# sea-with-sakura/ViT-of-Pytorch

Hardware: AMD Instinct MI355X
Metric: images/sec training step, ViT-B/16 224px bf16, 1/2/4/8 MI355X (higher is better)
Workload: dtype bf16; 1 GPU; ViT-B16 @224 train step (fwd+CE+bwd+SGD-momentum/OneCycleLR); model=ViT-B16, image_size=224, per_gpu_batch=256, global_batch=256, seq_len=197, num_classes=1000, parallelism=dp1, step_launch=eager

## Files before the change

### include/vit_hip.h

```cpp
#ifndef VIT_HIP_H_
#define VIT_HIP_H_

#include <stdint.h>

#ifdef __cplusplus
extern "C" {
#endif

typedef void* vit_stream_t;

enum vit_status {
  VIT_OK = 0,
  VIT_ERR_INVALID_ARG = 1,
  VIT_ERR_HIP = 2,
  VIT_ERR_UNSUPPORTED = 3,
};

const char* vit_last_error(void);
int vit_abi_version(void);
const char* vit_build_id(void);

enum vit_layout { VIT_K_CONTIG = 0, VIT_MN_CONTIG = 1 };

typedef struct vit_dropout {
// ... 84 lines not shown
                      const float* mean, const float* rstd, const float* gamma,
                      const float* dres, int64_t lddres, float* dx, int64_t lddx,
                      void* dx_bf16, int64_t lddxb, float* partial, float* dgamma_dbeta,
                      float* dx_colsum, int32_t accumulate_params, int64_t rows, int64_t D,
                      const vit_dropout* dx_dropout, vit_stream_t stream);

int vit_attention_fwd(const void* qkv, void* o, float* lse, int64_t B, int64_t N, int64_t H,
                      int64_t hd, float scale, vit_stream_t stream);
int vit_attention_bwd(const void* qkv, const void* o, const void* dout, const float* lse, void* dqkv,
                      float* bias_partial, int64_t B, int64_t N, int64_t H, int64_t hd, float scale,
                      vit_stream_t stream);
int vit_attention_fwd_rows(const void* qkv, void* o, float* lse, int64_t B, int64_t N, int64_t H, int64_t hd,
                           float scale, int64_t q_rows, vit_stream_t stream);
int vit_attention_bwd_rows(const void* qkv, const void* o, const void* dout, const float* lse, void* dqkv,
                           float* bias_partial, int64_t B, int64_t N, int64_t H, int64_t hd, float scale,
                           int64_t q_rows, vit_stream_t stream);
int64_t vit_attention_bias_rows(int64_t N, int64_t hd, int32_t path);
int64_t vit_attention_workspace_elems(int64_t B, int64_t N, int64_t H, int32_t path);
int vit_attention_fwd_ex(const void* qkv, void* o, float* lse, int64_t B, int64_t N, int64_t H, int64_t hd,
                         float scale, int64_t q_rows, int32_t path, vit_stream_t stream);
int vit_attention_bwd_ex(const void* qkv, const void* o, const void* dout, const float* lse, void* dqkv,
                         float* bias_partial, int64_t B, int64_t N, int64_t H, int64_t hd, float scale,
                         int64_t q_rows, int32_t path, float* workspace, vit_stream_t stream);

int vit_attention_fwd_varlen(const void* q, int64_t ldq, const void* k, int64_t ldk, const void* v, int64_t ldv,
                             void* o, int64_t ldo, const int32_t* cu_q, int64_t B, int64_t max_q, int64_t Nkv,
                             int64_t H, int64_t hd, float scale, vit_stream_t stream);

int vit_im2col(const float* x, void* out, int64_t B, int64_t img, int64_t P, int64_t Kpad,
               vit_stream_t stream);
int vit_im2col_hw(const float* x, void* out, int64_t B, int64_t H, int64_t W, int64_t Ph, int64_t Pw, int64_t Kpad,
                  vit_stream_t stream);

int vit_preprocess_u8(const uint8_t* images, int64_t B, int64_t H, int64_t W, int64_t image_stride,
                      const uint8_t* flips, int64_t out_h, int64_t out_w, const float* mean_std, float* out,
                      vit_stream_t stream);

enum vit_image_layout { VIT_IMAGES_HWC = 0, VIT_IMAGES_CHW = 1 };
int vit_preprocess_u8_gather(const uint8_t* images, int64_t n_images, int32_t layout, int64_t H, int64_t W,
                             int64_t image_stride, const int64_t* index, int64_t B, const uint8_t* flips,
                             int64_t out_h, int64_t out_w, const float* mean_std, float* out,
                             const int64_t* labels_in, int64_t* labels_out, vit_stream_t stream);

int vit_preprocess_u8_ragged(const uint8_t* bytes, int64_t n_bytes, const int64_t* geom, int64_t n_images,
                             const int64_t* index, int64_t B, const uint8_t* flips, int64_t out_h, int64_t out_w,
                             const float* mean_std, float* out, const int64_t* labels_in, int64_t* labels_out,
// ... 132 lines not shown
```

### vit-of-pytorch_amd/vitmi/_lib.py

```python
from __future__ import annotations

import ctypes
import os

_HERE = os.path.dirname(os.path.abspath(__file__))
LIB_PATH = os.environ.get("VITMI_LIB") or os.path.join(_HERE, "libvit_hip.so")

c_i64 = ctypes.c_int64
c_i32 = ctypes.c_int32
c_f32 = ctypes.c_float
c_vp = ctypes.c_void_p

ABI_VERSION = 24

K_CONTIG, MN_CONTIG = 0, 1
(EPI_F32, EPI_BF16, EPI_BIAS_BF16, EPI_BIAS_GELU, EPI_BIAS_RESID_F32, EPI_GELU_BWD, EPI_PATCH, EPI_SPLITK,
 EPI_BIAS_GELU_DGELU, EPI_MUL_BF16) = range(10)


class Dropout(ctypes.Structure):
    _fields_ = [("p", c_f32), ("site", ctypes.c_uint32), ("seed", ctypes.c_uint64), ("offset", ctypes.c_uint64),
                ("row_stride", c_i64)]


# ... 62 lines not shown
    "vit_cls_mse": (c_i32, [c_vp, c_i64, c_vp, c_i64, c_i64, c_i64, c_vp, c_vp, c_vp, c_vp]),
    "vit_cls_mse_bwd": (c_i32, [c_vp, c_i64, c_vp, c_i64, c_i64, c_vp, c_vp]),
    "vit_router_head_fwd": (c_i32, [c_vp, c_vp, c_i32, c_vp, c_i64, c_i64, c_i32, c_i64, c_i32, c_f32, c_vp, c_vp, c_vp,
                                    c_vp, c_vp, c_vp, c_vp]),
    "vit_router_head_bwd": (c_i32, [c_vp, c_vp, c_vp, c_vp, c_vp, c_vp, c_f32, c_i64, c_i64, c_i32, c_i64, c_i32, c_vp,
                                    c_vp]),
    "vit_splitk_reduce": (c_i32, [c_vp, c_i64, c_i64, c_i64, c_i64, c_vp, c_i64, c_i64, c_i32, c_vp]),
    "vit_layernorm_fwd": (c_i32, [c_vp, c_i64, c_vp, c_vp, c_vp, c_i64, c_i32, c_vp, c_vp, c_i64, c_i64, c_f32, c_vp]),
    "vit_layernorm_bwd_partial_rows": (c_i64, [c_i64]),
    "vit_layernorm_bwd_blocks": (c_i64, [c_i64]),
    "vit_layernorm_bwd": (c_i32, [c_vp, c_i64, c_i32, c_vp, c_i64, c_vp, c_vp, c_vp, c_vp, c_i64, c_vp, c_i64,
                                  c_vp, c_i64, c_vp, c_vp, c_vp, c_i32, c_i64, c_i64, ctypes.POINTER(Dropout),
                                  c_vp]),
    "vit_attention_fwd": (c_i32, [c_vp, c_vp, c_vp, c_i64, c_i64, c_i64, c_i64, c_f32, c_vp]),
    "vit_attention_bwd": (c_i32, [c_vp, c_vp, c_vp, c_vp, c_vp, c_vp, c_i64, c_i64, c_i64, c_i64, c_f32, c_vp]),
    "vit_attention_fwd_rows": (c_i32, [c_vp, c_vp, c_vp, c_i64, c_i64, c_i64, c_i64, c_f32, c_i64, c_vp]),
    "vit_attention_bwd_rows": (c_i32, [c_vp, c_vp, c_vp, c_vp, c_vp, c_vp, c_i64, c_i64, c_i64, c_i64, c_f32, c_i64,
                                       c_vp]),
    "vit_attention_bias_rows": (c_i64, [c_i64, c_i64, c_i32]),
    "vit_attention_workspace_elems": (c_i64, [c_i64, c_i64, c_i64, c_i32]),
    "vit_attention_fwd_ex": (c_i32, [c_vp, c_vp, c_vp, c_i64, c_i64, c_i64, c_i64, c_f32, c_i64, c_i32, c_vp]),
    "vit_attention_bwd_ex": (c_i32, [c_vp, c_vp, c_vp, c_vp, c_vp, c_vp, c_i64, c_i64, c_i64, c_i64, c_f32, c_i64,
                                     c_i32, c_vp, c_vp]),
    "vit_im2col": (c_i32, [c_vp, c_vp, c_i64, c_i64, c_i64, c_i64, c_vp]),
    "vit_im2col_hw": (c_i32, [c_vp, c_vp, c_i64, c_i64, c_i64, c_i64, c_i64, c_i64, c_vp]),
    "vit_preprocess_u8": (c_i32, [c_vp, c_i64, c_i64, c_i64, c_i64, c_vp, c_i64, c_i64, c_vp, c_vp, c_vp]),
    "vit_preprocess_u8_gather": (c_i32, [c_vp, c_i64, c_i32, c_i64, c_i64, c_i64, c_vp, c_i64, c_vp, c_i64, c_i64, c_vp,
                                         c_vp, c_vp, c_vp, c_vp]),
    "vit_preprocess_u8_ragged": (c_i32, [c_vp, c_i64, c_vp, c_i64, c_vp, c_i64, c_vp, c_i64, c_i64, c_vp, c_vp, c_vp,
                                         c_vp, c_vp]),
    "vit_preprocess_u8_ragged_crop": (c_i32, [c_vp, c_i64, c_vp, c_i64, c_vp, c_i64, c_vp, c_vp, c_i64, c_i64, c_vp,
                                              c_vp, c_vp, c_vp, c_vp]),
    "vit_mix_batch": (c_i32, [c_vp, c_vp, c_i64, c_i64, c_i64, c_vp, c_vp, c_vp, c_vp]),
    "vit_embed_grad": (c_i32, [c_vp, c_i64, c_i64, c_i64, c_vp, c_vp, c_vp, ctypes.POINTER(Dropout), c_vp]),
    "vit_embed_grad_accum": (c_i32, [c_vp, c_i64, c_i64, c_i64, c_vp, c_vp, c_vp, ctypes.POINTER(Dropout), c_i32,
                                     c_vp]),
    "vit_dropout_mask": (c_i32, [ctypes.POINTER(Dropout), c_i64, c_i64, c_i64, c_vp, c_i64, c_vp]),
    "vit_colsum_partial_rows": (c_i64, [c_i64]),
    "vit_colsum": (c_i32, [c_vp, c_i32, c_i64, c_i64, c_i64, c_vp, c_vp, c_i32, c_vp]),
    "vit_gemm_f32": (c_i32, [c_i64, c_i64, c_i64, c_vp, c_i64, c_i32, c_vp, c_i64, c_i32, c_vp, c_i64, c_vp, c_i32,
                             c_vp]),
    "vit_cross_entropy": (c_i32, [c_vp, c_vp, c_i64, c_i64, c_vp, c_f32, c_vp, c_vp]),
    "vit_cross_entropy_soft": (c_i32, [c_vp, c_vp, c_vp, c_vp, c_f32, c_i64, c_i64, c_vp, c_f32, c_vp, c_vp]),
    "vit_sgd_step": (c_i32, [c_vp, c_vp, c_vp, c_vp, c_i64, c_f32, c_f32, c_f32, c_i32, c_vp]),
    "vit_cast_f32_bf16": (c_i32, [c_vp, c_vp, c_i64, c_vp]),
    "vit_cast_pad_rows": (c_i32, [c_vp, c_i64, c_i64, c_vp, c_i64, c_vp]),
    "vit_axpby": (c_i32, [c_vp, c_vp, c_i64, c_f32, c_f32, c_vp]),
# ... 78 lines not shown
```

### vit-of-pytorch_amd/vitmi/engine.py

```python
from __future__ import annotations

import math
import os
from collections import OrderedDict
from dataclasses import dataclass

import torch

from . import ops, wgrad
from ._lib import (EPI_BF16, EPI_BIAS_BF16, EPI_BIAS_GELU_DGELU, EPI_BIAS_RESID_F32, EPI_MUL_BF16, EPI_PATCH,
                   K_CONTIG, MN_CONTIG)
from .wgrad import Spec

ALIGN = 64


def _rup(x, m):
    return (x + m - 1) // m * m


_NBUF = 2

_WGRAD_TARGET = int(os.environ.get("VIT_WGRAD_TARGET", "256"))

# ... 139 lines not shown
        self.g = [z(Tp, M) for _ in range(L)]
        self.lncls = z(b, D, dt=f)
        self.muf = z(b, dt=f)
        self.rsf = z(b, dt=f)
        self.logits = z(b, cfg.num_classes, dt=f)
        self.dh = z(Tp, D, dt=f)
        self.dhb = [z(Tp, D), z(Tp, D)]
        self.dg = [z(Tp, M), z(Tp, M)]
        self.dyln = z(Tp, D)
        self.dO = z(Tp, D)
        self.dqkv = [z(Tp, 3 * D), z(Tp, 3 * D)]
        self.dlncls = z(b, D, dt=f)
        self.dlogits = z(b, cfg.num_classes, dt=f)
        self.row_stats = z(b, 3, dt=f)
        self.lnparts = [z(ops.layernorm_bwd_blocks(T), 3 * D, dt=f) for _ in range(_NBUF)]
        self.gelu_parts = [z(-(-T // 128), M, dt=f) for _ in range(_NBUF)]
        self.attn_bias_rows = ops.attention_bias_rows(N, D // H)
        self.qkv_bparts = [z(b * self.attn_bias_rows, 3 * D, dt=f) for _ in range(_NBUF)]
        nws = ops.attention_workspace_elems(b, N, H)
        self.attn_ws = z(nws, dt=f) if nws else None
        bp = _rup(b, 64)
        self.bp = bp
        self.c_o, self.c_ln2, self.c_dh, self.c_dh2, self.c_dyln = (z(bp, D) for _ in range(5))
        self.c_g, self.c_gp, self.c_dg = (z(bp, M) for _ in range(3))
        self.c_mu2, self.c_rs2 = z(b, dt=f), z(b, dt=f)
        self._cfg, self._dev = cfg, dev
        self.dhb_l = self.dg_l = self.dqkv_l = None

    def defer_bufs(self):
        if self.dhb_l is None:
            cfg = self._cfg
            D, M, L = cfg.emb_dim, cfg.mlp_dim, cfg.num_layers
            z = lambda *s: torch.zeros(*s, device=self._dev, dtype=torch.bfloat16)
            self.dhb_l = self.dhb + [z(self.Tp, D) for _ in range(2 * L - 1)]
            self.dg_l = self.dg + [z(self.Tp, M) for _ in range(max(L - 2, 0))]
            self.dqkv_l = self.dqkv + [z(self.Tp, 3 * D) for _ in range(max(L - 2, 0))]
        return self.dhb_l, self.dg_l, self.dqkv_l


class _BiasReducer:

    def __init__(self, eng, a, accumulate=False):
        self.eng = eng
        self.a = a
        self.accumulate = accumulate
        self.D = eng.cfg.emb_dim
# ... 101 lines not shown
        D, L = cfg.emb_dim, cfg.num_layers
        M = cfg.mlp_dim
        bf = torch.bfloat16
        self.wqkv = torch.zeros(L, D, 3 * D, device=self.dev, dtype=bf)
        self.bqkv = torch.zeros(L, 3 * D, device=self.dev)
        kp = _rup(cfg.patch_k, 64)
        self.wconv = torch.zeros(D, kp, device=self.dev, dtype=torch.bfloat16) if kp != cfg.patch_k else None
        self._acts = {}
        self._mirror_sig = None
        o = [self.off(self.lname(i, "norm1.weight")) for i in range(L)]
        self.layer_stride = o[0] - o[1] if L > 1 else 0
        assert all(o[i] == o[0] - i * self.layer_stride for i in range(L))
        self._ws = None
        self.step_id = 0
        self.grad_ready_hook = None
        self.grad_ready_finish = None
        self.overlap_wgrad = os.environ.get("VITMI_OVERLAP", "0") == "1"
        self.group_wgrad = os.environ.get("VITMI_GROUP_WGRAD", "1") != "0"
        v = os.environ.get("VITMI_WGRAD_DEFER", "all")
        self.wgrad_defer = L if v == "all" else int(v)
        self._wgrad_tables = {}
        self.prune_last = os.environ.get("VITMI_PRUNE_LAST", "1") != "0"
        self._pruned = False
        self._side = None
        self._ev_pool, self._ev_next = [], 0
        self.probe = None
        self.probe_wgrad = None
        self.drop_seed = (torch.initial_seed() * 0x9E3779B97F4A7C15 + 0x632BE59BD9B4E019) & (2**64 - 1)
        self._drop_offset = 0
        self._drop = None

    def _event(self):
        if self._ev_next == len(self._ev_pool):
            self._ev_pool.append(torch.cuda.Event())
        ev = self._ev_pool[self._ev_next]
        self._ev_next += 1
        return ev

    def pv(self, name, buf=None):
        return self.layout.view(self.flat if buf is None else buf, name)

    def off(self, name):
        return self.layout.offsets[name]

    def lname(self, i, s):
        return f"transformer.encoder_layers.{i}.{s}"
# ... 55 lines not shown
        b = x.shape[0]
        a = self.acts(b)
        D, M, H, N, L = cfg.emb_dim, cfg.mlp_dim, cfg.num_heads, cfg.tokens, cfg.num_layers
        hd = D // H
        T = a.T
        mv = self.mirror
        f = self.flat
        if dropout_p and dropout_p > 0.0:
            if not dropout_p < 1.0:
                raise ValueError(f"dropout probability has to be in [0, 1), got {dropout_p}")
            self._drop_offset += 1
            self._drop = (float(dropout_p), self.drop_seed, self._drop_offset)
        else:
            self._drop = None
        dd = self._dd
        ops.im2col_hw(x, a.patches, b, *cfg.image_hw, *cfg.patch_hw, a.kpad)
        wconv = self.wconv if self.wconv is not None else mv[self.off("embedding.weight"):]
        ops.gemm(a.patches, wconv, a.h[0], T, D, a.kpad, a_layout=K_CONTIG, b_layout=K_CONTIG, lda=a.kpad,
                 ldb=a.kpad, ldc=D, epilogue=EPI_PATCH, bias=f[self.off("embedding.bias"):],
                 aux=f[self.off("transformer.pos_embedding.pos_embedding"):], ldaux=D,
                 aux2=f[self.off("cls_token"):], tokens=N, dropout=dd(0))
        scale = 1.0 / math.sqrt(hd)
        self._pruned = self.prune_last and self._drop is None
        for i in range(L):
            ln = lambda s: self.off(self.lname(i, s))
            ops.layernorm_fwd(a.h[i], D, f[ln("norm1.weight"):], f[ln("norm1.bias"):], a.ln1[i], D, a.mu1[i],
                              a.rs1[i], T, D)
            ops.gemm(a.ln1[i], self.wqkv[i], a.qkv[i], T, 3 * D, D, a_layout=K_CONTIG, b_layout=MN_CONTIG, lda=D,
                     ldb=3 * D, ldc=3 * D, epilogue=EPI_BIAS_BF16, bias=self.bqkv[i])
            last = self._pruned and i == L - 1
            ops.attention_fwd(a.qkv[i], a.o[i], a.lse[i], b, N, H, hd, scale, q_rows=1 if last else None,
                              path=self.attn_fwd_path)
            if last:
                self._forward_last_cls(a, i, b)
                break
            ops.gemm(a.o[i], mv[ln("attn.out.weight"):], a.hm[i], T, D, D, a_layout=K_CONTIG, b_layout=MN_CONTIG,
                     lda=D, ldb=D, ldc=D, epilogue=EPI_BIAS_RESID_F32, bias=f[ln("attn.out.bias"):], aux=a.h[i],
                     ldaux=D, dropout=dd(1 + 3 * i))
            ops.layernorm_fwd(a.hm[i], D, f[ln("norm2.weight"):], f[ln("norm2.bias"):], a.ln2[i], D, a.mu2[i],
                              a.rs2[i], T, D)
            wgrad.timed(self.probe, (), ops.gemm, a.ln2[i], mv[ln("mlp.fc1.weight"):], a.gp[i], T, M, D,
                        a_layout=K_CONTIG, b_layout=K_CONTIG, lda=D, ldb=D, ldc=M, epilogue=EPI_BIAS_GELU_DGELU,
                        bias=f[ln("mlp.fc1.bias"):], C2=a.g[i], ldc2=M, dropout=dd(2 + 3 * i))
            ops.gemm(a.g[i], mv[ln("mlp.fc2.weight"):], a.h[i + 1], T, D, M, a_layout=K_CONTIG, b_layout=K_CONTIG,
                     lda=M, ldb=M, ldc=D, epilogue=EPI_BIAS_RESID_F32, bias=f[ln("mlp.fc2.bias"):], aux=a.hm[i],
                     ldaux=D, dropout=dd(3 + 3 * i))
        ops.layernorm_fwd(a.h[L], N * D, f[self.off("transformer.norm.weight"):], f[self.off("transformer.norm.bias"):],
                          a.lncls, D, a.muf, a.rsf, b, D)
        C = cfg.num_classes
        ops.gemm_f32(b, C, D, a.lncls, D, False, f[self.off("classifier.weight"):], D, True, a.logits, C,
                     bias=f[self.off("classifier.bias"):])
        self.step_id += 1
        self._last_b = b
        return a.logits

# ... 14 lines not shown
                 lda=M, ldb=M, ldc=S, epilogue=EPI_BIAS_RESID_F32, bias=f[ln("mlp.fc2.bias"):], aux=a.hm[i], ldaux=S)

    def _backward_last_cls(self, a, i, b, g, wq, bias):
        cfg = self.cfg
        D, M, N = cfg.emb_dim, cfg.mlp_dim, cfg.tokens
        S = N * D
        f, mv = self.flat, self.mirror
        gv = lambda name: g[self.off(self.lname(i, name)):]
        bp = a.bp
        wq.single(Spec(a.c_dh, D, a.c_g, M, D, M, gv("mlp.fc2.weight"), M), K=bp)
        gpart = bias.buf("gelu", a.gelu_parts)
        w2 = mv[self.off(self.lname(i, "mlp.fc2.weight")):]
        kw = dict(a_layout=K_CONTIG, b_layout=MN_CONTIG, lda=D, ldb=M, ldc=M, epilogue=EPI_MUL_BF16, aux=a.c_gp,
                  ldaux=M, col_partial=gpart)
        ops.gemm(a.c_dh, w2, a.c_dg, b, M, D, **kw)
        tiles_m = ops.gemm_partial_rows(a.c_dh, w2, a.c_dg, b, M, D, **kw)
        bias.reduce(gpart, tiles_m, M, M, (gv("mlp.fc1.bias"),))
        wq.single(Spec(a.c_dg, M, a.c_ln2, D, M, D, gv("mlp.fc1.weight"), D), K=bp)
        ops.gemm(a.c_dg, mv[self.off(self.lname(i, "mlp.fc1.weight")):], a.c_dyln, b, D, M, a_layout=K_CONTIG,
                 b_layout=MN_CONTIG, lda=M, ldb=D, ldc=D, epilogue=EPI_BF16)
        bias.ln_bwd(a.c_dyln, D, a.hm[i], S, a.c_mu2, a.c_rs2, f[self.off(self.lname(i, "norm2.weight")):], a.dh, S, b,
                    gv("norm2.weight"), gv("attn.out.bias"), dres=a.dh, lddres=S, dx_bf16=a.c_dh2, lddxb=D)
        wq.single(Spec(a.c_o, D, a.c_dh2, D, D, D, gv("attn.out.weight"), D), K=bp)
        ops.zero_(a.dO)
        ops.gemm(a.c_dh2, mv[self.off(self.lname(i, "attn.out.weight")):], a.dO, b, D, D, a_layout=K_CONTIG,
                 b_layout=K_CONTIG, lda=D, ldb=D, ldc=S, epilogue=EPI_BF16)

    def forward_exact(self, x: torch.Tensor):
        cfg = self.cfg
        if x.dim() != 4 or x.shape[1] != 3 or tuple(x.shape[2:]) != cfg.image_hw:
            raise ValueError(f"expected input [b, 3, {cfg.image_hw[0]}, {cfg.image_hw[1]}], got {tuple(x.shape)}")
        x = x.to(self.dev, torch.float32).contiguous()
        b = x.shape[0]
        D, M, H, N, L, C = cfg.emb_dim, cfg.mlp_dim, cfg.num_heads, cfg.tokens, cfg.num_layers, cfg.num_classes
        hd = D // H
        T, kp = b * N, cfg.patch_k
        f = self.flat
        e = lambda *shape: torch.empty(*shape, device=self.dev)
        fv = lambda name: f[self.off(name):]
        patches = e(T, kp)
        ops.im2col_hw_f32(x, patches, b, *cfg.image_hw, *cfg.patch_hw, kp)
        h = e(T, D)
        ops.gemm_f32(T, D, kp, patches, kp, False, fv("embedding.weight"), kp, True, h, D, bias=fv("embedding.bias"))
        ops.embed_fwd_f32(h, b, N, D, fv("transformer.pos_embedding.pos_embedding"), fv("cls_token"))
        y, qkv, o, u = e(T, D), e(T, 3 * D), e(T, D), e(T, M)
        mu, rs = e(T), e(T)
        for i in range(L):
# ... 120 lines not shown
                w2 = mv[ln("mlp.fc2.weight"):]
                kw = dict(a_layout=K_CONTIG, b_layout=MN_CONTIG, lda=D, ldb=M, ldc=M, epilogue=EPI_MUL_BF16, aux=a.gp[i],
                          ldaux=M, col_partial=gpart)
                ops.gemm(dhb, w2, dg, T, M, D, **kw)
                tiles_m = ops.gemm_partial_rows(dhb, w2, dg, T, M, D, **kw)
                bias.reduce(gpart, tiles_m, M, M, (gv(self.lname(i, "mlp.fc1.bias")),))
                wq.push(Spec(dg, M, a.ln2[i], D, M, D, gv(self.lname(i, "mlp.fc1.weight")), D),
                        done=lambda k=li: release("dg", k))
                ops.gemm(dg, mv[ln("mlp.fc1.weight"):], a.dyln, T, D, M, a_layout=K_CONTIG, b_layout=MN_CONTIG, lda=M,
                         ldb=D, ldc=D, epilogue=EPI_BF16)
                wb = (wb + 1) % nd
                acquire("dhb", wb)
                dhb = dhbs[wb]
                bias.ln_bwd(a.dyln, D, a.hm[i], D, a.mu2[i], a.rs2[i], f[ln("norm2.weight"):], a.dh, D, T,
                            gv(self.lname(i, "norm2.weight")), gv(self.lname(i, "attn.out.bias")),
                            dres=a.dh, lddres=D, dx_bf16=dhb, lddxb=D, dx_dropout=dd(1 + 3 * i))
                wq.push(Spec(a.o[i], D, dhb, D, D, D, gv(self.lname(i, "attn.out.weight")), D),
                        done=lambda k=wb: release("dhb", k), hold=True)
                ops.gemm(dhb, mv[ln("attn.out.weight"):], a.dO, T, D, D, a_layout=K_CONTIG, b_layout=K_CONTIG, lda=D,
                         ldb=D, ldc=D, epilogue=EPI_BF16)
            dqkv = dqkvs[li]
            acquire("dqkv", li)
            qpart = bias.buf("qkv", a.qkv_bparts)
            ops.attention_bwd(a.qkv[i], a.o[i], a.dO, a.lse[i], dqkv, b, N, H, hd, scale, bias_partial=qpart,
                              q_rows=1 if pruned and i == L - 1 else None, workspace=a.attn_ws)
            qo = ln("attn.query.weight")
            zs = ln("attn.key.weight") - qo
            qb = ln("attn.query.bias")
            bias.reduce(qpart, b * a.attn_bias_rows, 3 * D, 3 * D, (g[qb:], g[qb + zs:], g[qb + 2 * zs:]), seg=D)
            wq.push(Spec(a.ln1[i], D, dqkv, 3 * D, D, D, g[qo:], D, batch=3, b_bs=D, out_bs=zs),
                    done=lambda k=li: release("dqkv", k))
            wq.end_layer(i)
            ops.gemm(dqkv, self.wqkv[i], a.dyln, T, D, 3 * D, a_layout=K_CONTIG, b_layout=K_CONTIG, lda=3 * D,
                     ldb=3 * D, ldc=D, epilogue=EPI_BF16)
            wb = (wb + 1) % nd
            acquire("dhb", wb)
            bias.ln_bwd(a.dyln, D, a.h[i], D, a.mu1[i], a.rs1[i], f[ln("norm1.weight"):], a.dh, D, T,
                        gv(self.lname(i, "norm1.weight")), gv(self.lname(i - 1, "mlp.fc2.bias")) if i > 0 else None,
                        dres=a.dh, lddres=D, dx_bf16=dhbs[wb], lddxb=D,
                        dx_dropout=dd(3 + 3 * (i - 1)) if i > 0 else dd(0))
            fire(self.layout.buckets[L - i])
        wq.push(Spec(dhbs[wb], D, a.patches, a.kpad, D, cfg.patch_k, gv("embedding.weight"), cfg.patch_k))
        wq.finish()
        ops.embed_grad(a.dh, b, N, D, gv("transformer.pos_embedding.pos_embedding"), gv("cls_token"),
                       gv("embedding.bias"), dropout=dd(0), accumulate=accumulate)
        fire(self.layout.buckets[-1])
        bias.flush()
        if overlap:
            main.wait_stream(side)
        return g
```

### vit-of-pytorch_amd/vitmi/ops.py

```python
from __future__ import annotations

import ctypes

import torch

from . import _lib
from ._lib import COLSUM_BATCH_MAX, Dropout, GemmArgs, check

BF16 = torch.bfloat16
F32 = torch.float32


def lib():
    return _lib.load()


def _stream():
    return ctypes.c_void_p(torch.cuda.current_stream().cuda_stream)


def _p(t):
    return ctypes.c_void_p(0 if t is None else t.data_ptr())


# ... 124 lines not shown
def attention_workspace_elems(B, N, H, path=ATTN_AUTO):
    return int(lib().vit_attention_workspace_elems(B, N, H, path))


def attention_fwd(qkv, o, lse, B, N, H, hd, scale, q_rows=None, path=ATTN_AUTO):
    _chk(qkv, BF16, "qkv")
    _chk(o, BF16, "o")
    _chk(lse, F32, "lse")
    check(lib().vit_attention_fwd_ex(_p(qkv), _p(o), _p(lse), B, N, H, hd, scale, N if q_rows is None else q_rows,
                                     path, _stream()), "vit_attention_fwd")


def attention_bwd(qkv, o, dout, lse, dqkv, B, N, H, hd, scale, bias_partial=None, q_rows=None, path=ATTN_AUTO,
                  workspace=None):
    _chk(workspace, F32, "workspace")
    need = attention_workspace_elems(B, N, H, path)
    if need and (workspace is None or workspace.numel() < need):
        if workspace is not None:
            raise ValueError(f"attention workspace has {workspace.numel()} floats, needs {need}")
        workspace = torch.empty(need, device=qkv.device, dtype=F32)
    check(lib().vit_attention_bwd_ex(_p(qkv), _p(o), _p(dout), _p(lse), _p(dqkv), _p(bias_partial), B, N, H, hd,
                                     scale, N if q_rows is None else q_rows, path, _p(workspace if need else None),
                                     _stream()), "vit_attention_bwd")


def im2col(x, out, B, img, P, Kpad):
    _chk(x, F32, "x")
    _chk(out, BF16, "out")
    check(lib().vit_im2col(_p(x), _p(out), B, img, P, Kpad, _stream()), "vit_im2col")


def im2col_hw(x, out, B, H, W, Ph, Pw, Kpad):
    _chk(x, F32, "x")
    _chk(out, BF16, "out")
    check(lib().vit_im2col_hw(_p(x), _p(out), B, H, W, Ph, Pw, Kpad, _stream()), "vit_im2col_hw")


def preprocess_u8(images, out, flips=None, mean=(0.5, 0.5, 0.5), std=(0.5, 0.5, 0.5)):
    _chk(images, torch.uint8, "images")
    _chk(out, F32, "out")
    _chk(flips, torch.uint8, "flips")
    if images.dim() != 4 or images.shape[3] != 3 or out.dim() != 4 or out.shape[1] != 3:
        raise ValueError(f"preprocess_u8: images [B,H,W,3] -> out [B,3,h,w], got {tuple(images.shape)} -> "
                         f"{tuple(out.shape)}")
    B, H, W, _ = images.shape
    if out.shape[0] != B or (flips is not None and flips.numel() != B):
# ... 399 lines not shown

def adamw_ema_update(p, g, m, v, p_bf16, ema, chunks, table, lr, beta1, beta2, eps, wd, ema_decay, write_grad):
    for t, name in ((p, "p"), (g, "g"), (m, "m"), (v, "v"), (ema, "ema"), (table, "table")):
        _chk(t, F32, name)
    _chk(p_bf16, BF16, "p_bf16")
    if chunks.is_cuda or chunks.dtype != torch.int64 or not chunks.is_contiguous() or not chunks.is_pinned():
        raise ValueError("adamw_ema_update: chunks must be a contiguous int64 tensor in pinned host memory")
    check(lib().vit_adamw_ema_update(_p(p), _p(g), _p(m), _p(v), _p(p_bf16), _p(ema), _p(chunks), chunks.numel() // 3,
                                     _p(table), 1.0 - lr * wd, beta1, beta2, 1.0 - beta1, 1.0 - beta2, eps,
                                     0.0 if ema is None else 1.0 - ema_decay, int(write_grad), _stream()),
          "vit_adamw_ema_update")


def scale_by_coef(g, n, coef):
    check(lib().vit_scale_by_coef(_p(g), n, _p(coef), _stream()), "vit_scale_by_coef")


def zero_(t):
    if not t.is_contiguous():
        raise ValueError("zero_: contiguous tensor expected")
    check(lib().vit_zero(_p(t), t.numel() * t.element_size(), _stream()), "vit_zero")


def _splitk_model(tiles, slots, tile, K, slab_elems):
    smax = max(1, min((K // 64) // 8, 32))
    t_tile = 2.0 * tile * tile * K / 4.0e12
    slab = 2.0 * slab_elems * 4 / 5.0e12
    best, best_t = 1, None
    for s in range(1, smax + 1):
        t = -(-tiles * s // slots) * t_tile / s + s * slab
        if best_t is None or t < best_t * (1 - 1e-9):
            best, best_t = s, t
    return best


def splitk_factor_group(shapes, K, cus=256):
    tiles = sum(-(-M // 256) * -(-N // 256) * b for M, N, b in shapes)
    return _splitk_model(tiles, cus, 256, K, sum(M * N * b for M, N, b in shapes))


def gemm_splitk_group(members):
    if not 1 <= len(members) <= 4:
        raise ValueError("gemm_splitk_group: 1 to 4 members")
    arr = (GemmArgs * len(members))()
    for i, (A, B, C, M, N, K, kw) in enumerate(members):
        _chk(A, BF16, "A")
        _chk(B, BF16, "B")
        arr[i] = _gemm_args(A, B, C, M, N, K, **kw)
    check(lib().vit_gemm_splitk_group(arr, len(members), _stream()), "vit_gemm_splitk_group")


GEMM_TABLE_MAX = 128


class GemmGroupTable:

    def __init__(self, members):
        n = len(members)
        if not 1 <= n <= GEMM_TABLE_MAX:
            raise ValueError(f"GemmGroupTable: 1 to {GEMM_TABLE_MAX} members")
        arr = (GemmArgs * n)()
# ... 48 lines not shown
```

### vit-of-pytorch_amd/vitmi/wgrad.py

```python
from __future__ import annotations

from typing import NamedTuple

import torch

from . import ops
from ._lib import EPI_SPLITK, MN_CONTIG


class Spec(NamedTuple):
    A: torch.Tensor
    lda: int
    B: torch.Tensor
    ldb: int
    M: int
    N: int
    out: object
    ldo: int
    batch: int = 1
    a_bs: int = 0
    b_bs: int = 0
    out_bs: int = 0
    accumulate: object = False

# ... 58 lines not shown
        jobs += _reduce_jobs(sp, s, w)
    return views, members, jobs


def single(sp, K, alloc=None, target=256, probe=None):
    s = ops.splitk_factor(sp.M, sp.N, K, sp.batch, target)
    ws = _alloc(alloc, sp, _slabs([sp], [s]))
    timed(probe, _tail(probe, [sp], K, False), ops.gemm, sp.A, sp.B, ws, sp.M, sp.N, K, **_gemm_kw(sp, s, sp.N))
    for job in _reduce_jobs(sp, s, ws):
        ops.splitk_reduce(*job)


def group(specs, K, common, alloc=None, target=256, probe=None):
    if common:
        splits = [ops.splitk_factor_group([(sp.M, sp.N, sp.batch) for sp in specs], K, target)] * len(specs)
    else:
        splits = [ops.splitk_factor(sp.M, sp.N, K, sp.batch, target) for sp in specs]
    _, members, jobs = plan(specs, K, splits, _alloc(alloc, specs[0], _slabs(specs, splits)))
    timed(probe, _tail(probe, specs, K, True), ops.gemm_splitk_group, members)
    ops.splitk_reduce_group(jobs)


def table(specs, K, tables, slot, alloc=None, target=256, probe=None):
    s = ops.splitk_factor_group([(sp.M, sp.N, sp.batch) for sp in specs], K, target)
    ws = _alloc(alloc, specs[0], _slabs(specs, [s] * len(specs))) if s > 1 else None
    jobs, o = [], 0
    for c0 in range(0, len(specs), ops.GEMM_TABLE_MAX):
        part = specs[c0:c0 + ops.GEMM_TABLE_MAX]
        key = (s, K, o, ws.data_ptr() if s > 1 else 0) + tuple(
            (sp.A.data_ptr(), sp.lda, sp.B.data_ptr(), sp.ldb, sp.M, sp.N, sp.out.data_ptr(), sp.ldo, sp.batch, sp.a_bs,
             sp.b_bs, sp.out_bs, bool(sp.accumulate)) for sp in part)
        ent = tables.get((slot, c0))
        if ent is None or ent[0] != key:
            _, members, red = plan(part, K, [s] * len(part), ws[o:] if s > 1 else None, table=True)
            ent = tables[(slot, c0)] = (key, ops.GemmGroupTable(members), red)
        timed(probe, _tail(probe, part, K, True), ent[1].launch)
        jobs += ent[2]
        o += _slabs(part, [s] * len(part)) if s > 1 else 0
    if jobs:
        ops.splitk_reduce_group(jobs)
```

Baseline: 7761 images/sec.

## Prune last-layer Q projection to CLS rows with dedicated CLS attention kernels

In the last transformer layer, only the CLS token's output is needed, so the QKV projection now computes K and V for all tokens but Q only for the CLS row. New single-query attention forward and backward kernels handle that layer. The backward pass likewise restricts the Q weight-gradient and the dX GEMM to the CLS rows, and drops the dO zeroing. Separately, the split-K cost model for table wgrad no longer charges a reduction slab when split is 1. The cost is new kernels and copy2d staging, plus dependence on the layout of the existing buffers.

```diff
diff --git a/include/vit_hip.h b/include/vit_hip.h
--- a/include/vit_hip.h
+++ b/include/vit_hip.h
@@ -130,6 +130,13 @@
 int vit_attention_bwd_ex(const void* qkv, const void* o, const void* dout, const float* lse, void* dqkv,
                          float* bias_partial, int64_t B, int64_t N, int64_t H, int64_t hd, float scale,
                          int64_t q_rows, int32_t path, float* workspace, vit_stream_t stream);
+
+int vit_attention_cls_supported(int64_t N, int64_t hd);
+int vit_attention_cls_fwd(const void* qkv, void* o, float* lse, int64_t B, int64_t N, int64_t H, int64_t hd,
+                          float scale, vit_stream_t stream);
+int vit_attention_cls_bwd(const void* qkv, const void* dout, const float* lse, void* dqkv, float* bias_partial,
+                          int64_t bias_rows, int64_t B, int64_t N, int64_t H, int64_t hd, float scale,
+                          vit_stream_t stream);
 
 int vit_attention_fwd_varlen(const void* q, int64_t ldq, const void* k, int64_t ldk, const void* v, int64_t ldv,
                              void* o, int64_t ldo, const int32_t* cu_q, int64_t B, int64_t max_q, int64_t Nkv,
diff --git a/vit-of-pytorch_amd/csrc/attention_cls.hip b/vit-of-pytorch_amd/csrc/attention_cls.hip
--- /dev/null
+++ b/vit-of-pytorch_amd/csrc/attention_cls.hip
@@ -0,0 +1,317 @@
+#include "common.h"
+
+namespace {
+
+constexpr int TPB = 256;
+constexpr int QPAD = 96;
+constexpr int64_t MAX_N = 1024;
+
+__device__ __forceinline__ void unpack8(const uint4& w, float* f) {
+  f[0] = __uint_as_float(w.x << 16); f[1] = __uint_as_float(w.x & 0xffff0000u);
+  f[2] = __uint_as_float(w.y << 16); f[3] = __uint_as_float(w.y & 0xffff0000u);
+  f[4] = __uint_as_float(w.z << 16); f[5] = __uint_as_float(w.z & 0xffff0000u);
+  f[6] = __uint_as_float(w.w << 16); f[7] = __uint_as_float(w.w & 0xffff0000u);
+}
+__device__ __forceinline__ float dot8(const uint4& w, const float* x) {
+  float f[8];
+  unpack8(w, f);
+  float s = f[0] * x[0];
+#pragma unroll
+  for (int e = 1; e < 8; ++e) s = fmaf(f[e], x[e], s);
+  return s;
+}
+__device__ __forceinline__ float round_bf(float x) { return bf2f(f2bf(x)); }
+
+__device__ __forceinline__ float block_sum(float v, float* red) {
+  v = wave_sum(v);
+  if ((threadIdx.x & 63) == 0) red[threadIdx.x >> 6] = v;
+  __syncthreads();
+  const float r = (red[0] + red[1]) + (red[2] + red[3]);
+  __syncthreads();
+  return r;
+}
+__device__ __forceinline__ float block_max(float v, float* red) {
+  v = wave_max(v);
+  if ((threadIdx.x & 63) == 0) red[threadIdx.x >> 6] = v;
+  __syncthreads();
+  const float r = fmaxf(fmaxf(red[0], red[1]), fmaxf(red[2], red[3]));
+  __syncthreads();
+  return r;
+}
+
+template <int HD>
+struct Geo {
+  static constexpr int CPK = HD / 8;
+  static constexpr int G = TPB / CPK;
+};
+template <int HD>
+size_t part_floats(int N) {
+  const size_t a = (size_t)N * Geo<HD>::CPK, b = (size_t)Geo<HD>::G * HD;
+  return a > b ? a : b;
+}
+inline int pad4(int n) { return (n + 3) & ~3; }
+
+template <int HD>
+__global__ __launch_bounds__(TPB) void attn_cls_fwd_kernel(const bf16_t* __restrict__ qkv, bf16_t* __restrict__ o,
+                                                           float* __restrict__ lse, int N, int npad, int H,
+                                                           float scale) {
+  constexpr int CPK = Geo<HD>::CPK, G = Geo<HD>::G;
+  extern __shared__ __attribute__((aligned(16))) float smem[];
+  float* qs = smem;
+  float* red = qs + QPAD;
+  float* sc = red + 8;
+  float* part = sc + npad;
+  const int tid = threadIdx.x, b = blockIdx.x / H, h = blockIdx.x % H;
+  const int D = H * HD;
+  const size_t ld = 3 * (size_t)D;
+  const bf16_t* base = qkv + (size_t)b * N * ld + (size_t)h * HD;
+  if (tid < HD) qs[tid] = bf2f(base[tid]);
+  __syncthreads();
+  const int g = tid / CPK, c = tid % CPK;
+  const bool active = g < G;
+  float qr[8];
+#pragma unroll
+  for (int e = 0; e < 8; ++e) qr[e] = qs[c * 8 + e];
+  if (active) {
+    const bf16_t* kp = base + D + c * 8;
+#pragma unroll 4
+    for (int j = g; j < N; j += G) {
+      const uint4 w = *reinterpret_cast<const uint4*>(kp + (size_t)j * ld);
+      part[j * CPK + c] = dot8(w, qr);
+    }
+  }
+  __syncthreads();
+  float m = -INFINITY;
+  for (int j = tid; j < N; j += TPB) {
+    float s = part[j * CPK];
+#pragma unroll
+    for (int k = 1; k < CPK; ++k) s += part[j * CPK + k];
+    s *= scale;
+    sc[j] = s;
+    m = fmaxf(m, s);
+  }
+  m = block_max(m, red);
+  float l = 0.0f;
+  for (int j = tid; j < N; j += TPB) {
+    const float p = expf(sc[j] - m);
+    l += p;
+    sc[j] = round_bf(p);
+  }
+  l = block_sum(l, red);
+  float acc[8] = {0.0f, 0.0f, 0.0f, 0.0f, 0.0f, 0.0f, 0.0f, 0.0f};
+  if (active) {
+    const bf16_t* vp = base + 2 * D + c * 8;
+#pragma unroll 4
+    for (int j = g; j < N; j += G) {
+      const uint4 w = *reinterpret_cast<const uint4*>(vp + (size_t)j * ld);
+      float v[8];
+      unpack8(w, v);
+      const float p = sc[j];
+#pragma unroll
+      for (int e = 0; e < 8; ++e) acc[e] = fmaf(p, v[e], acc[e]);
+    }
+#pragma unroll
+    for (int e = 0; e < 8; ++e) part[g * HD + c * 8 + e] = acc[e];
+  }
+  __syncthreads();
+  if (tid < HD) {
+    float s = part[tid];
+    for (int k = 1; k < G; ++k) s += part[k * HD + tid];
+    o[(size_t)b * N * D + (size_t)h * HD + tid] = f2bf(s / l);
+  }
+  if (tid == 0) lse[((size_t)b * H + h) * N] = m + logf(l);
+}
+
+template <int HD>
+__global__ __launch_bounds__(TPB) void attn_cls_bwd_kernel(const bf16_t* __restrict__ qkv,
+                                                           const bf16_t* __restrict__ dout,
+                                                           const float* __restrict__ lse, bf16_t* __restrict__ dqkv,
+                                                           float* __restrict__ bias_partial, int bias_rows, int N,
+                                                           int npad, int H, float scale) {
+  constexpr int CPK = Geo<HD>::CPK, G = Geo<HD>::G;
+  extern __shared__ __attribute__((aligned(16))) float smem[];
+  float* qs = smem;
+  float* dos = qs + QPAD;
+  float* red = dos + QPAD;
+  float* sp = red + 8;
+  float* sd = sp + npad;
+  float* partp = sd + npad;
+  float* parts = partp + (size_t)N * CPK;
+  const int tid = threadIdx.x, b = blockIdx.x / H, h = blockIdx.x % H;
+  const int D = H * HD;
+  const size_t ld = 3 * (size_t)D;
+  const size_t row0 = (size_t)b * N * ld + (size_t)h * HD;
+  const bf16_t* base = qkv + row0;
+  if (tid < HD) {
+    qs[tid] = bf2f(base[tid]);
+    dos[tid] = bf2f(dout[(size_t)b * N * D + (size_t)h * HD + tid]);
+  }
+  const float L = lse[((size_t)b * H + h) * N];
+  __syncthreads();
+  const int g = tid / CPK, c = tid % CPK;
+  const bool active = g < G;
+  float qr[8], dr[8];
+#pragma unroll
+  for (int e = 0; e < 8; ++e) {
+    qr[e] = qs[c * 8 + e];
+    dr[e] = dos[c * 8 + e];
+  }
+  const bf16_t* kp = base + D + c * 8;
+  if (active) {
+#pragma unroll 4
+    for (int j = g; j < N; j += G) {
+      const uint4 kw = *reinterpret_cast<const uint4*>(kp + (size_t)j * ld);
+      const uint4 vw = *reinterpret_cast<const uint4*>(kp + D + (size_t)j * ld);
+      parts[j * CPK + c] = dot8(kw, qr);
+      partp[j * CPK + c] = dot8(vw, dr);
+    }
+  }
+  __syncthreads();
+  float dl = 0.0f;
+  for (int j = tid; j < N; j += TPB) {
+    float s = parts[j * CPK], dp = partp[j * CPK];
+#pragma unroll
+    for (int k = 1; k < CPK; ++k) {
+      s += parts[j * CPK + k];
+      dp += partp[j * CPK + k];
+    }
+    const float p = expf(s * scale - L);
+    sp[j] = p;
+    sd[j] = dp;
+    dl = fmaf(p, dp, dl);
+  }
+  const float delta = block_sum(dl, red);
+  float sum_p = 0.0f, sum_ds = 0.0f;
+  for (int j = tid; j < N; j += TPB) {
+    const float p = sp[j];
+    const float pb = round_bf(p), dsb = round_bf(p * (sd[j] - delta));
+    sp[j] = pb;
+    sd[j] = dsb;
+    sum_p += pb;
+    sum_ds += dsb;
+  }
+  sum_p = block_sum(sum_p, red);
+  sum_ds = block_sum(sum_ds, red);
+  float acc[8] = {0.0f, 0.0f, 0.0f, 0.0f, 0.0f, 0.0f, 0.0f, 0.0f};
+  if (active) {
+    bf16_t* dkp = dqkv + row0 + D + c * 8;
+#pragma unroll 2
+    for (int j = g; j < N; j += G) {
+      const uint4 kw = *reinterpret_cast<const uint4*>(kp + (size_t)j * ld);
+      float k[8];
+      unpack8(kw, k);
+      const float pb = sp[j], dsb = sd[j];
+      uint4 dk, dv;
+      dk.x = pack2bf(scale * (dsb * qr[0]), scale * (dsb * qr[1]));
+      dk.y = pack2bf(scale * (dsb * qr[2]), scale * (dsb * qr[3]));
+      dk.z = pack2bf(scale * (dsb * qr[4]), scale * (dsb * qr[5]));
+      dk.w = pack2bf(scale * (dsb * qr[6]), scale * (dsb * qr[7]));
+      dv.x = pack2bf(pb * dr[0], pb * dr[1]);
+      dv.y = pack2bf(pb * dr[2], pb * dr[3]);
+      dv.z = pack2bf(pb * dr[4], pb * dr[5]);
+      dv.w = pack2bf(pb * dr[6], pb * dr[7]);
+      *reinterpret_cast<uint4*>(dkp + (size_t)j * ld) = dk;
+      *reinterpret_cast<uint4*>(dkp + D + (size_t)j * ld) = dv;
+#pragma unroll
+      for (int e = 0; e < 8; ++e) acc[e] = fmaf(dsb, k[e], acc[e]);
+    }
+#pragma unroll
+    for (int e = 0; e < 8; ++e) parts[g * HD + c * 8 + e] = acc[e];
+  }
+  __syncthreads();
+  if (tid < HD) {
+    float s = parts[tid];
+    for (int k = 1; k < G; ++k) s += parts[k * HD + tid];
+    const float dq = scale * s;
+    dqkv[row0 + tid] = f2bf(dq);
+    if (bias_partial) {
+      float* bp = bias_partial + (size_t)b * bias_rows * ld + (size_t)h * HD + tid;
+      bp[0] = dq;
+      bp[D] = scale * (sum_ds * qs[tid]);
+      bp[2 * D] = sum_p * dos[tid];
+      for (int r = 1; r < bias_rows; ++r) {
+        bp[r * ld] = 0.0f;
+        bp[r * ld + D] = 0.0f;
+        bp[r * ld + 2 * D] = 0.0f;
+      }
+    }
+  }
+}
+
+template <int HD>
+hipError_t launch_fwd(const void* qkv, void* o, float* lse, int B, int N, int H, float scale, hipStream_t s) {
+  const int npad = pad4(N);
+  const size_t lds = (QPAD + 8 + npad + part_floats<HD>(N)) * sizeof(float);
+  auto kern = attn_cls_fwd_kernel<HD>;
+  if (lds > 64 * 1024) (void)hipFuncSetAttribute((const void*)kern, hipFuncAttributeMaxDynamicSharedMemorySize, (int)lds);
+  hipLaunchKernelGGL(kern, dim3(B * H), dim3(TPB), lds, s, (const bf16_t*)qkv, (bf16_t*)o, lse, N, npad, H, scale);
+  return hipGetLastError();
+}
+
+template <int HD>
+hipError_t launch_bwd(const void* qkv, const void* dout, const float* lse, void* dqkv, float* bias_partial,
+                      int bias_rows, int B, int N, int H, float scale, hipStream_t s) {
+  const int npad = pad4(N);
+  const size_t lds = (2 * QPAD + 8 + 2 * npad + (size_t)N * Geo<HD>::CPK + part_floats<HD>(N)) * sizeof(float);
+  auto kern = attn_cls_bwd_kernel<HD>;
+  if (lds > 64 * 1024) (void)hipFuncSetAttribute((const void*)kern, hipFuncAttributeMaxDynamicSharedMemorySize, (int)lds);
+  hipLaunchKernelGGL(kern, dim3(B * H), dim3(TPB), lds, s, (const bf16_t*)qkv, (const bf16_t*)dout, lse, (bf16_t*)dqkv,
+                     bias_partial, bias_rows, N, npad, H, scale);
+  return hipGetLastError();
+}
+
+bool supported(int64_t N, int64_t hd) { return (hd == 32 || hd == 64 || hd == 80) && N >= 1 && N <= MAX_N; }
+bool aligned16(const void* p) { return ((uintptr_t)p & 15) == 0; }
+
+int check(const char* what, int64_t B, int64_t N, int64_t H, int64_t hd) {
+  VIT_CHECK_ARG(B >= 1 && H >= 1 && N >= 1 && hd >= 1, "%s: bad sizes B=%lld N=%lld H=%lld hd=%lld", what, (long long)B,
+                (long long)N, (long long)H, (long long)hd);
+  VIT_CHECK_ARG(B * H <= 0x7fffffff && H * hd <= (1 << 20), "%s: B=%lld H=%lld hd=%lld too large", what, (long long)B,
+                (long long)H, (long long)hd);
+  if (!supported(N, hd)) {
+    vit::set_error("%s: N=%lld hd=%lld unsupported (hd 32, 64 or 80, N <= %lld)", what, (long long)N, (long long)hd,
+                   (long long)MAX_N);
+    return VIT_ERR_UNSUPPORTED;
+  }
+  return VIT_OK;
+}
+
+}
+
+extern "C" int vit_attention_cls_supported(int64_t N, int64_t hd) { return supported(N, hd) ? 1 : 0; }
+
+extern "C" int vit_attention_cls_fwd(const void* qkv, void* o, float* lse, int64_t B, int64_t N, int64_t H, int64_t hd,
+                                     float scale, vit_stream_t stream) {
+  const int st = check("vit_attention_cls_fwd", B, N, H, hd);
+  if (st) return st;
+  VIT_CHECK_ARG(qkv && o && lse, "vit_attention_cls_fwd: null pointer");
+  VIT_CHECK_ARG(aligned16(qkv), "vit_attention_cls_fwd: qkv must be 16-byte aligned");
+  hipStream_t s = (hipStream_t)stream;
+  hipError_t e;
+  switch (hd) {
+    case 32: e = launch_fwd<32>(qkv, o, lse, (int)B, (int)N, (int)H, scale, s); break;
+    case 64: e = launch_fwd<64>(qkv, o, lse, (int)B, (int)N, (int)H, scale, s); break;
+    default: e = launch_fwd<80>(qkv, o, lse, (int)B, (int)N, (int)H, scale, s); break;
+  }
+  return vit::check_hip(e, "vit_attention_cls_fwd launch");
+}
+
+extern "C" int vit_attention_cls_bwd(const void* qkv, const void* dout, const float* lse, void* dqkv,
+                                     float* bias_partial, int64_t bias_rows, int64_t B, int64_t N, int64_t H,
+                                     int64_t hd, float scale, vit_stream_t stream) {
+  const int st = check("vit_attention_cls_bwd", B, N, H, hd);
+  if (st) return st;
+  VIT_CHECK_ARG(qkv && dout && lse && dqkv, "vit_attention_cls_bwd: null pointer");
+  VIT_CHECK_ARG(aligned16(qkv) && aligned16(dqkv), "vit_attention_cls_bwd: qkv / dqkv must be 16-byte aligned");
+  VIT_CHECK_ARG(!bias_partial || (bias_rows >= 1 && bias_rows <= 1024), "vit_attention_cls_bwd: bias_rows=%lld",
+                (long long)bias_rows);
+  hipStream_t s = (hipStream_t)stream;
+  const int br = (int)bias_rows;
+  hipError_t e;
+  switch (hd) {
+    case 32: e = launch_bwd<32>(qkv, dout, lse, dqkv, bias_partial, br, (int)B, (int)N, (int)H, scale, s); break;
+    case 64: e = launch_bwd<64>(qkv, dout, lse, dqkv, bias_partial, br, (int)B, (int)N, (int)H, scale, s); break;
+    default: e = launch_bwd<80>(qkv, dout, lse, dqkv, bias_partial, br, (int)B, (int)N, (int)H, scale, s); break;
+  }
+  return vit::check_hip(e, "vit_attention_cls_bwd launch");
+}
diff --git a/vit-of-pytorch_amd/vitmi/_lib.py b/vit-of-pytorch_amd/vitmi/_lib.py
--- a/vit-of-pytorch_amd/vitmi/_lib.py
+++ b/vit-of-pytorch_amd/vitmi/_lib.py
@@ -108,7 +108,10 @@
     "vit_attention_fwd_ex": (c_i32, [c_vp, c_vp, c_vp, c_i64, c_i64, c_i64, c_i64, c_f32, c_i64, c_i32, c_vp]),
     "vit_attention_bwd_ex": (c_i32, [c_vp, c_vp, c_vp, c_vp, c_vp, c_vp, c_i64, c_i64, c_i64, c_i64, c_f32, c_i64,
                                      c_i32, c_vp, c_vp]),
-    "vit_im2col": (c_i32, [c_vp, c_vp, c_i64, c_i64, c_i64, c_i64, c_vp]),
+    "vit_attention_cls_supported": (c_i32, [c_i64, c_i64]),
+    "vit_attention_cls_fwd": (c_i32, [c_vp, c_vp, c_vp, c_i64, c_i64, c_i64, c_i64, c_f32, c_vp]),
+    "vit_attention_cls_bwd": (c_i32, [c_vp, c_vp, c_vp, c_vp, c_vp, c_i64, c_i64, c_i64, c_i64, c_i64, c_f32, c_vp]),
+    "vit_im2col":(c_i32, [c_vp, c_vp, c_i64, c_i64, c_i64, c_i64, c_vp]),
     "vit_im2col_hw": (c_i32, [c_vp, c_vp, c_i64, c_i64, c_i64, c_i64, c_i64, c_i64, c_vp]),
     "vit_preprocess_u8": (c_i32, [c_vp, c_i64, c_i64, c_i64, c_i64, c_vp, c_i64, c_i64, c_vp, c_vp, c_vp]),
     "vit_preprocess_u8_gather": (c_i32, [c_vp, c_i64, c_i32, c_i64, c_i64, c_i64, c_vp, c_i64, c_vp, c_i64, c_i64, c_vp,
diff --git a/vit-of-pytorch_amd/vitmi/engine.py b/vit-of-pytorch_amd/vitmi/engine.py
--- a/vit-of-pytorch_amd/vitmi/engine.py
+++ b/vit-of-pytorch_amd/vitmi/engine.py
@@ -185,6 +185,7 @@
         bp = _rup(b, 64)
         self.bp = bp
         self.c_o, self.c_ln2, self.c_dh, self.c_dh2, self.c_dyln = (z(bp, D) for _ in range(5))
+        self.c_ln1, self.c_dq = z(bp, D), z(bp, D)
         self.c_g, self.c_gp, self.c_dg = (z(bp, M) for _ in range(3))
         self.c_mu2, self.c_rs2 = z(b, dt=f), z(b, dt=f)
         self._cfg, self._dev = cfg, dev
@@ -332,6 +333,8 @@
         self._wgrad_tables = {}
         self.prune_last = os.environ.get("VITMI_PRUNE_LAST", "1") != "0"
         self._pruned = False
+        self.prune_q = os.environ.get("VITMI_PRUNE_Q", "1") != "0"
+        self._prune_q = False
         self._side = None
         self._ev_pool, self._ev_next = [], 0
         self.probe = None
@@ -433,15 +436,23 @@
                  aux2=f[self.off("cls_token"):], tokens=N, dropout=dd(0))
         scale = 1.0 / math.sqrt(hd)
         self._pruned = self.prune_last and self._drop is None
+        self._prune_q = self._pruned and self.prune_q and ops.attention_cls_supported(N, hd)
         for i in range(L):
             ln = lambda s: self.off(self.lname(i, s))
             ops.layernorm_fwd(a.h[i], D, f[ln("norm1.weight"):], f[ln("norm1.bias"):], a.ln1[i], D, a.mu1[i],
                               a.rs1[i], T, D)
-            ops.gemm(a.ln1[i], self.wqkv[i], a.qkv[i], T, 3 * D, D, a_layout=K_CONTIG, b_layout=MN_CONTIG, lda=D,
-                     ldb=3 * D, ldc=3 * D, epilogue=EPI_BIAS_BF16, bias=self.bqkv[i])
             last = self._pruned and i == L - 1
-            ops.attention_fwd(a.qkv[i], a.o[i], a.lse[i], b, N, H, hd, scale, q_rows=1 if last else None,
-                              path=self.attn_fwd_path)
+            if last and self._prune_q:
+                kw = dict(a_layout=K_CONTIG, b_layout=MN_CONTIG, ldb=3 * D, epilogue=EPI_BIAS_BF16)
+                ops.gemm(a.ln1[i], self.wqkv[i].view(-1)[D:], a.qkv[i].view(-1)[D:], T, 2 * D, D, lda=D, ldc=3 * D,
+                         bias=self.bqkv[i][D:], **kw)
+                ops.gemm(a.ln1[i], self.wqkv[i], a.qkv[i], b, D, D, lda=N * D, ldc=3 * N * D, bias=self.bqkv[i], **kw)
+                ops.attention_cls_fwd(a.qkv[i], a.o[i], a.lse[i], b, N, H, hd, scale)
+            else:
+                ops.gemm(a.ln1[i], self.wqkv[i], a.qkv[i], T, 3 * D, D, a_layout=K_CONTIG, b_layout=MN_CONTIG, lda=D,
+                         ldb=3 * D, ldc=3 * D, epilogue=EPI_BIAS_BF16, bias=self.bqkv[i])
+                ops.attention_fwd(a.qkv[i], a.o[i], a.lse[i], b, N, H, hd, scale, q_rows=1 if last else None,
+                                  path=self.attn_fwd_path)
             if last:
                 self._forward_last_cls(a, i, b)
                 break
@@ -502,7 +513,8 @@
         bias.ln_bwd(a.c_dyln, D, a.hm[i], S, a.c_mu2, a.c_rs2, f[self.off(self.lname(i, "norm2.weight")):], a.dh, S, b,
                     gv("norm2.weight"), gv("attn.out.bias"), dres=a.dh, lddres=S, dx_bf16=a.c_dh2, lddxb=D)
         wq.single(Spec(a.c_o, D, a.c_dh2, D, D, D, gv("attn.out.weight"), D), K=bp)
-        ops.zero_(a.dO)
+        if not self._prune_q:
+            ops.zero_(a.dO)
         ops.gemm(a.c_dh2, mv[self.off(self.lname(i, "attn.out.weight")):], a.dO, b, D, D, a_layout=K_CONTIG,
                  b_layout=K_CONTIG, lda=D, ldb=D, ldc=S, epilogue=EPI_BF16)
 
@@ -669,17 +681,33 @@
             dqkv = dqkvs[li]
             acquire("dqkv", li)
             qpart = bias.buf("qkv", a.qkv_bparts)
-            ops.attention_bwd(a.qkv[i], a.o[i], a.dO, a.lse[i], dqkv, b, N, H, hd, scale, bias_partial=qpart,
-                              q_rows=1 if pruned and i == L - 1 else None, workspace=a.attn_ws)
+            pq = self._prune_q and i == L - 1
+            if pq:
+                ops.attention_cls_bwd(a.qkv[i], a.dO, a.lse[i], dqkv, b, N, H, hd, scale, bias_partial=qpart,
+                                      bias_rows=a.attn_bias_rows)
+            else:
+                ops.attention_bwd(a.qkv[i], a.o[i], a.dO, a.lse[i], dqkv, b, N, H, hd, scale, bias_partial=qpart,
+                                  q_rows=1 if pruned and i == L - 1 else None, workspace=a.attn_ws)
             qo = ln("attn.query.weight")
             zs = ln("attn.key.weight") - qo
             qb = ln("attn.query.bias")
             bias.reduce(qpart, b * a.attn_bias_rows, 3 * D, 3 * D, (g[qb:], g[qb + zs:], g[qb + 2 * zs:]), seg=D)
-            wq.push(Spec(a.ln1[i], D, dqkv, 3 * D, D, D, g[qo:], D, batch=3, b_bs=D, out_bs=zs),
-                    done=lambda k=li: release("dqkv", k))
+            if pq:
+                ops.copy2d(a.c_ln1, D * 2, a.ln1[i], N * D * 2, D * 2, b)
+                ops.copy2d(a.c_dq, D * 2, dqkv, 3 * N * D * 2, D * 2, b)
+                wq.single(Spec(a.c_ln1, D, a.c_dq, D, D, D, g[qo:], D), K=a.bp)
+                wq.push(Spec(a.ln1[i], D, dqkv.view(-1)[D:], 3 * D, D, D, g[qo + zs:], D, batch=2, b_bs=D, out_bs=zs),
+                        done=lambda k=li: release("dqkv", k))
+            else:
+                wq.push(Spec(a.ln1[i], D, dqkv, 3 * D, D, D, g[qo:], D, batch=3, b_bs=D, out_bs=zs),
+                        done=lambda k=li: release("dqkv", k))
             wq.end_layer(i)
-            ops.gemm(dqkv, self.wqkv[i], a.dyln, T, D, 3 * D, a_layout=K_CONTIG, b_layout=K_CONTIG, lda=3 * D,
-                     ldb=3 * D, ldc=D, epilogue=EPI_BF16)
+            kw = dict(a_layout=K_CONTIG, b_layout=K_CONTIG, ldb=3 * D, epilogue=EPI_BF16)
+            if pq:
+                ops.gemm(dqkv.view(-1)[D:], self.wqkv[i].view(-1)[D:], a.dyln, T, D, 2 * D, lda=3 * D, ldc=D, **kw)
+                ops.gemm(dqkv, self.wqkv[i], a.dyln, b, D, 3 * D, lda=3 * N * D, ldc=N * D, **kw)
+            else:
+                ops.gemm(dqkv, self.wqkv[i], a.dyln, T, D, 3 * D, lda=3 * D, ldc=D, **kw)
             wb = (wb + 1) % nd
             acquire("dhb", wb)
             bias.ln_bwd(a.dyln, D, a.h[i], D, a.mu1[i], a.rs1[i], f[ln("norm1.weight"):], a.dh, D, T,
diff --git a/vit-of-pytorch_amd/vitmi/ops.py b/vit-of-pytorch_amd/vitmi/ops.py
--- a/vit-of-pytorch_amd/vitmi/ops.py
+++ b/vit-of-pytorch_amd/vitmi/ops.py
@@ -170,6 +170,27 @@
     check(lib().vit_attention_bwd_ex(_p(qkv), _p(o), _p(dout), _p(lse), _p(dqkv), _p(bias_partial), B, N, H, hd,
                                      scale, N if q_rows is None else q_rows, path, _p(workspace if need else None),
                                      _stream()), "vit_attention_bwd")
+
+
+def attention_cls_supported(N, hd):
+    return bool(lib().vit_attention_cls_supported(N, hd))
+
+
+def attention_cls_fwd(qkv, o, lse, B, N, H, hd, scale):
+    _chk(qkv, BF16, "qkv")
+    _chk(o, BF16, "o")
+    _chk(lse, F32, "lse")
+    check(lib().vit_attention_cls_fwd(_p(qkv), _p(o), _p(lse), B, N, H, hd, scale, _stream()), "vit_attention_cls_fwd")
+
+
+def attention_cls_bwd(qkv, dout, lse, dqkv, B, N, H, hd, scale, bias_partial=None, bias_rows=1):
+    _chk(qkv, BF16, "qkv")
+    _chk(dout, BF16, "dout")
+    _chk(lse, F32, "lse")
+    _chk(dqkv, BF16, "dqkv")
+    _chk(bias_partial, F32, "bias_partial")
+    check(lib().vit_attention_cls_bwd(_p(qkv), _p(dout), _p(lse), _p(dqkv), _p(bias_partial), bias_rows, B, N, H, hd,
+                                      scale, _stream()), "vit_attention_cls_bwd")
 
 
 def im2col(x, out, B, img, P, Kpad):
@@ -615,21 +636,21 @@
     check(lib().vit_zero(_p(t), t.numel() * t.element_size(), _stream()), "vit_zero")
 
 
-def _splitk_model(tiles, slots, tile, K, slab_elems):
+def _splitk_model(tiles, slots, tile, K, slab_elems, direct=False):
     smax = max(1, min((K // 64) // 8, 32))
     t_tile = 2.0 * tile * tile * K / 4.0e12
     slab = 2.0 * slab_elems * 4 / 5.0e12
     best, best_t = 1, None
     for s in range(1, smax + 1):
-        t = -(-tiles * s // slots) * t_tile / s + s * slab
+        t = -(-tiles * s // slots) * t_tile / s + (0 if direct and s == 1 else s) * slab
         if best_t is None or t < best_t * (1 - 1e-9):
             best, best_t = s, t
     return best
 
 
-def splitk_factor_group(shapes, K, cus=256):
+def splitk_factor_group(shapes, K, cus=256, direct=False):
     tiles = sum(-(-M // 256) * -(-N // 256) * b for M, N, b in shapes)
-    return _splitk_model(tiles, cus, 256, K, sum(M * N * b for M, N, b in shapes))
+    return _splitk_model(tiles, cus, 256, K, sum(M * N * b for M, N, b in shapes), direct)
 
 
 def gemm_splitk_group(members):
diff --git a/vit-of-pytorch_amd/vitmi/wgrad.py b/vit-of-pytorch_amd/vitmi/wgrad.py
--- a/vit-of-pytorch_amd/vitmi/wgrad.py
+++ b/vit-of-pytorch_amd/vitmi/wgrad.py
@@ -104,7 +104,7 @@
 
 
 def table(specs, K, tables, slot, alloc=None, target=256, probe=None):
-    s = ops.splitk_factor_group([(sp.M, sp.N, sp.batch) for sp in specs], K, target)
+    s = ops.splitk_factor_group([(sp.M, sp.N, sp.batch) for sp in specs], K, target, direct=True)
     ws = _alloc(alloc, specs[0], _slabs(specs, [s] * len(specs))) if s > 1 else None
     jobs, o = [], 0
     for c0 in range(0, len(specs), ops.GEMM_TABLE_MAX):
```

After: 7792 images/sec, median of 6. About the same (+0.4%).
